# andimarafioti/faster-qwen3-tts

Hardware: AMD Instinct MI355X
Metric: real-time factor (audio s / wall s), Qwen3-TTS-12Hz-0.6B voice-clone streaming chunk_size=8; p50 TTFA in ttfa_ms_p50 (higher is better)
Workload: dtype bf16

## Files before the change

### faster-qwen3-tts_amd/csrc/decode_kernels.cuh

```cuda
#pragma once
#include "fq3_common.cuh"

namespace fq3 {

enum { PRO_PLAIN = 0, PRO_NORM = 1, PRO_COMBINE = 2 };
enum { EPI_STORE = 0, EPI_RESIDUAL = 1, EPI_SWIGLU = 2 };

constexpr int kHeadDim = 128;
constexpr int kKeysPerTile = 64;
constexpr int kMaxWorkers = 8;
constexpr int kPartStride = kHeadDim + 4;


struct GemvArgs {
    const void* W; int N; int K;
    const void* x;
    const void* norm_w; float eps;
    const void* bias;
    void* y;
    const void* res;
    void* xn_out;
    int up_off;
    const float* part; int n_part; int rep;
    const void* x2; void* y2; const void* res2; size_t part_stride2;
// ... 352 lines not shown
        l[h] = xrow_sum(l[h] * w);
#pragma unroll
        for (int i = 0; i < 8; ++i) o[h][i] = xrow_sum(o[h][i] * w);
        m[h] = M;
    }
    if (sub == 0) {
#pragma unroll
        for (int h = 0; h < REP; ++h) {
#pragma unroll
            for (int i = 0; i < 8; ++i) wo[wave][h][c * 8 + i] = o[h][i];
            if (c == 0) { wm[wave][h] = m[h]; wl[wave][h] = l[h]; }
        }
    }
    __syncthreads();
    for (int e = tid; e < REP * HD; e += 256) {
        const int h = e / HD, d = e - h * HD;
        float M = fmaxf(fmaxf(wm[0][h], wm[1][h]), fmaxf(wm[2][h], wm[3][h]));
        float num = 0.f, den = 0.f;
#pragma unroll
        for (int w = 0; w < 4; ++w) {
            const float ww = __expf(wm[w][h] - M);
            num = fmaf(ww, wo[w][h][d], num);
            den = fmaf(ww, wl[w][h], den);
        }
        float* p = a.part + (((size_t)g * kMaxWorkers + s) * REP + h) * kPartStride;
        p[d] = num;
        if (d == 0) { p[HD] = M; p[HD + 1] = den; }
    }
}

template <typename T, int REP, bool PAGED>
__global__ __launch_bounds__(256) void attn_decode_kernel(AttnArgs a) { attn_decode_body<T, REP, PAGED>(a); }

template <typename T>
__device__ __forceinline__ void attn_pred_body(const AttnArgs& a, int head) {
    constexpr int HD = kHeadDim;
    const int g = head / a.rep, hh = head - g * a.rep;
    const int lane = threadIdx.x & 63, sub = lane >> 4, c = lane & 15;
    const int pos = a.pos_imm;
    const T* qkv = reinterpret_cast<const T*>(a.qkv);
    const int q_dim = a.n_kv * a.rep * HD, kv_dim = a.n_kv * HD;
    T* kc = reinterpret_cast<T*>(a.kcache) + (size_t)g * a.max_seq * HD;
    T* vc = reinterpret_cast<T*>(a.vcache) + (size_t)g * a.max_seq * HD;
    Raw8<T> qraw, knraw, vnraw, qwraw, kwraw, kr[4], vr[4];
    ldraw<false>(qraw, qkv + (size_t)head * HD + c * 8);
    ldraw<false>(knraw, qkv + q_dim + (size_t)g * HD + c * 8);
    ldraw<false>(vnraw, qkv + q_dim + kv_dim + (size_t)g * HD + c * 8);
    ldraw<false>(qwraw, reinterpret_cast<const T*>(a.q_norm_w) + c * 8);
    ldraw<false>(kwraw, reinterpret_cast<const T*>(a.k_norm_w) + c * 8);
    const f32x4 cs0 = *reinterpret_cast<const f32x4*>(a.cos_row + ((c * 8) & 63)), cs1 = *reinterpret_cast<const f32x4*>(a.cos_row + ((c * 8 + 4) & 63));
    const f32x4 sn0 = *reinterpret_cast<const f32x4*>(a.sin_row + ((c * 8) & 63)), sn1 = *reinterpret_cast<const f32x4*>(a.sin_row + ((c * 8 + 4) & 63));
#pragma unroll
    for (int i = 0; i < 4; ++i) {
        int key = i * 4 + sub;
        key = key < a.max_seq ? key : a.max_seq - 1;
        ldraw<false>(kr[i], kc + (size_t)key * HD + c * 8);
        ldraw<false>(vr[i], vc + (size_t)key * HD + c * 8);
    }
    __builtin_amdgcn_sched_barrier(0);
    const float sgn = c < 8 ? -1.f : 1.f;
    const float cs[8] = {cs0.x, cs0.y, cs0.z, cs0.w, cs1.x, cs1.y, cs1.z, cs1.w};
    const float sn[8] = {sgn * sn0.x, sgn * sn0.y, sgn * sn0.z, sgn * sn0.w, sgn * sn1.x, sgn * sn1.y, sgn * sn1.z, sgn * sn1.w};
    auto norm_rope = [&](const Raw8<T>& raw, const Raw8<T>& wraw, float (&out)[8]) {
        float x[8], w[8];
        unpack(raw, x); unpack(wraw, w);
        float ss = 0.f;
#pragma unroll
        for (int i = 0; i < 8; ++i) ss = fmaf(x[i], x[i], ss);
        ss = row16_sum(ss);
        const float rs = 1.0f / sqrtf(ss / (float)HD + a.eps);
#pragma unroll
        for (int i = 0; i < 8; i += 2) {
            float u = x[i] * rs, v = x[i + 1] * rs;
            DT<T>::rnd2(u, v);
            u *= w[i]; v *= w[i + 1];
            DT<T>::rnd2(u, v);
            x[i] = u; x[i + 1] = v;
        }
#pragma unroll
        for (int i = 0; i < 8; i += 2) {
            float a0 = x[i] * cs[i], a1 = x[i + 1] * cs[i + 1];
            float b0 = row16_xor8(x[i]) * sn[i], b1 = row16_xor8(x[i + 1]) * sn[i + 1];
            DT<T>::rnd2(a0, a1); DT<T>::rnd2(b0, b1);
            float r0 = a0 + b0, r1 = a1 + b1;
            DT<T>::rnd2(r0, r1);
            out[i] = r0; out[i + 1] = r1;
        }
    };
    float qr[8], knew[8], vnew[8];
    norm_rope(qraw, qwraw, qr);
    norm_rope(knraw, kwraw, knew);
    unpack(vnraw, vnew);
    if (hh == 0 && sub == 0) {
        DT<T>::st8(kc + (size_t)pos * HD + c * 8, knew);
        DT<T>::st8(vc + (size_t)pos * HD + c * 8, vnew);
    }
    float sc[5];
#pragma unroll
    for (int i = 0; i < 4; ++i) {
        float kf[8], s = 0.f;
        unpack(kr[i], kf);
#pragma unroll
        for (int d = 0; d < 8; ++d) s = fmaf(qr[d], kf[d], s);
        s = row16_sum(s);
        sc[i] = (i * 4 + sub < pos) ? s * a.scale : -INFINITY;
    }
    {
        float s = 0.f;
#pragma unroll
        for (int d = 0; d < 8; ++d) s = fmaf(qr[d], knew[d], s);
        s = row16_sum(s);
        sc[4] = sub == 0 ? s * a.scale : -INFINITY;
    }
    const float mx = wave_max(fmaxf(fmaxf(fmaxf(sc[0], sc[1]), fmaxf(sc[2], sc[3])), sc[4]));
    float p[5], lsum = 0.f, o[8];
#pragma unroll
    for (int i = 0; i < 5; ++i) { p[i] = __expf(sc[i] - mx); lsum += p[i]; }
    lsum = wave_sum(lsum) * (1.0f / 16.0f);
#pragma unroll
    for (int d = 0; d < 8; ++d) o[d] = p[4] * vnew[d];
#pragma unroll
    for (int i = 0; i < 4; ++i) {
        float vf[8];
        if (!(i * 4 + sub < pos)) zero(vr[i]);
        unpack(vr[i], vf);
#pragma unroll
        for (int d = 0; d < 8; ++d) o[d] = fmaf(p[i], vf[d], o[d]);
    }
    const float inv = 1.0f / lsum;
#pragma unroll
    for (int d = 0; d < 8; ++d) o[d] = xrow_sum(o[d]) * inv;
    if (sub == 0) DT<T>::st8(reinterpret_cast<T*>(a.out) + (size_t)head * HD + c * 8, o);
}

// ... 79 lines not shown
            float s = 0.f;
#pragma unroll
            for (int d = 0; d < 8; ++d) s = fmaf(qr[d], kf[i][d], s);
            s = row16_sum(s);
            sc[i] = (i * 4 + sub < pos) ? s * a.scale : -INFINITY;
        }
        {
            float s = 0.f;
#pragma unroll
            for (int d = 0; d < 8; ++d) s = fmaf(qr[d], knew[d], s);
            s = row16_sum(s);
            sc[4] = sub == 0 ? s * a.scale : -INFINITY;
        }
        const float mx = wave_max(fmaxf(fmaxf(fmaxf(sc[0], sc[1]), fmaxf(sc[2], sc[3])), sc[4]));
        float p[5], lsum = 0.f, o[8];
#pragma unroll
        for (int i = 0; i < 5; ++i) { p[i] = __expf(sc[i] - mx); lsum += p[i]; }
        lsum = wave_sum(lsum) * (1.0f / 16.0f);
#pragma unroll
        for (int d = 0; d < 8; ++d) o[d] = p[4] * vnew[d];
#pragma unroll
        for (int i = 0; i < 4; ++i)
#pragma unroll
            for (int d = 0; d < 8; ++d) o[d] = fmaf(p[i], vf[i][d], o[d]);
        const float inv = 1.0f / lsum;
#pragma unroll
        for (int d = 0; d < 8; ++d) o[d] = xrow_sum(o[d]) * inv;
        if (sub == 0) DT<T>::st8(reinterpret_cast<T*>(a.out) + (size_t)(g * REP + h) * HD + c * 8, o);
    }
}

template <typename T>
__global__ __launch_bounds__(64) void attn_pred_kernel(AttnArgs a) { attn_pred_body<T>(a); }

template <typename T>
__global__ __launch_bounds__(256) void rmsnorm_kernel(const T* x, const T* w, T* y, int K, float eps) {
    __shared__ float red[8];
    float ss = 0.f;
    for (int e = threadIdx.x; e < K; e += 256) { const float v = DT<T>::ld(x + e); ss = fmaf(v, v, ss); }
    ss = block_sum<4>(ss, red);
    const float rs = 1.0f / sqrtf(ss / (float)K + eps);
    for (int e = threadIdx.x; e < K; e += 256)
        DT<T>::st(y + e, DT<T>::ld(w + e) * DT<T>::rnd(DT<T>::ld(x + e) * rs));
}

template <typename T>
__global__ void copy_kernel(T* dst, const T* src, int n) {
    const int i = blockIdx.x * blockDim.x + threadIdx.x;
    if (i < n) dst[i] = src[i];
}

struct DecodeState {
    int token, frame, pos, gen_step, done;
    int min_new, max_new, trailing_len, noise_frames, eos_id, max_seq, sup_lo, sup_hi;
    float t_temperature; int t_top_k; float t_top_p; int t_do_sample; float t_rep_penalty;
    float p_temperature; int p_top_k; float p_top_p; int p_do_sample;
    const void* trailing_text; const void* tts_pad; const void* talker_noise; const void* pred_noise;
    const void* past_hidden_init;
    int n_pad, rope_delta;
};

struct TeacherForcing { const int* forced; int* decisions; };

__device__ __forceinline__ int forced_or(const TeacherForcing* tf, int slot, int tok) {
    if (!tf) return tok;
    const int* forced = gptr(tf->forced); int* dec = gptr(tf->decisions);
    if (dec && threadIdx.x == 0) dec[slot] = tok;
    return forced ? forced[slot] : tok;
}

template <typename T>
__device__ __forceinline__ void frame_begin_body(DecodeState* st, const T* codec_emb, const T* past_hidden,
                                                 T* pred_in, int* codes, unsigned char* seen, int H, int G) {
    if (st->done) return;
    const int tok = st->token;
    if (tok == st->eos_id || st->frame >= st->max_new) {
        __syncthreads();
        if (threadIdx.x == 0) st->done = 1;
        return;
    }
    if (threadIdx.x == 0) { codes[(size_t)st->frame * G] = tok; seen[tok] = 1; }
    for (int e = threadIdx.x; e < H; e += 256) {
        pred_in[e] = past_hidden[e];
        pred_in[H + e] = codec_emb[(size_t)tok * H + e];
    }
}
template <typename T>
__global__ __launch_bounds__(256) void frame_begin_kernel(DecodeState* st, const T* codec_emb, const T* past_hidden,
                                                          T* pred_in, int* codes, unsigned char* seen, int H, int G) {
    frame_begin_body<T>(st, codec_emb, past_hidden, pred_in, codes, seen, H, G);
}

struct EmbTables { const void* t[32]; };

template <typename T, int G>
__device__ __forceinline__ void embed_sum_body(DecodeState* st, const EmbTables& tabs, const int* codes, T* x, int H,
                                               const float* cos_tab, const float* sin_tab, int rope_len,
                                               int rope_delta, float* rope_now) {
    const int done = st->done, frame = st->frame, pos = st->pos, gen_step = st->gen_step;
    const int trailing_len = st->trailing_len, max_seq = st->max_seq;
    const T* trailing = gptr(reinterpret_cast<const T*>(st->trailing_text));
    const T* pad = gptr(reinterpret_cast<const T*>(st->tts_pad));
    if (done) return;
    if (pos >= max_seq - 1) {
        __syncthreads();
        if (threadIdx.x == 0) { st->frame = frame + 1; st->done = 1; }
        return;
    }
    int ids[G];
#pragma unroll
    for (int gI = 0; gI < G; ++gI) ids[gI] = codes[(size_t)frame * G + gI];
    if (threadIdx.x < kHeadDim) {
        int rp = pos + rope_delta;
        rp = rp < 0 ? 0 : (rp >= rope_len ? rope_len - 1 : rp);
        const int i = threadIdx.x & 63;
        rope_now[threadIdx.x] = threadIdx.x < 64 ? cos_tab[(size_t)rp * 64 + i] : sin_tab[(size_t)rp * 64 + i];
    }
    const T* text = gen_step < trailing_len ? trailing + (size_t)gen_step * H : pad;
    for (int e0 = threadIdx.x * 8; e0 < H; e0 += 256 * 8) {
        Raw8<T> r[G], tr;
#pragma unroll
        for (int gI = 0; gI < G; ++gI) ldraw<false>(r[gI], reinterpret_cast<const T*>(tabs.t[gI]) + (size_t)ids[gI] * H + e0);
        ldraw<false>(tr, text + e0);
        float sum[8], f[8];
        unpack(r[0], sum);
#pragma unroll
        for (int gI = 1; gI < G; ++gI) {
            unpack(r[gI], f);
#pragma unroll
            for (int i = 0; i < 8; ++i) sum[i] += f[i];
        }
        unpack(tr, f);
#pragma unroll
        for (int i = 0; i < 8; ++i) DT<T>::st(x + e0 + i, DT<T>::rnd(sum[i]) + f[i]);
    }
}
template <typename T, int G>
__global__ __launch_bounds__(256) void embed_sum_kernel(DecodeState* st, EmbTables tabs, const int* codes, T* x, int H,
                                                        const float* cos_tab, const float* sin_tab, int rope_len,
                                                        int rope_delta, float* rope_now) {
    embed_sum_body<T, G>(st, tabs, codes, x, H, cos_tab, sin_tab, rope_len, rope_delta, rope_now);
}

}
// ... 1 lines not shown
```

### faster-qwen3-tts_amd/csrc/fq3_api.hip

```cpp
#define FQ3_SKINNY_EXTERN
#include "fq3_ctx.h"
#include "sampler.cuh"
#include "sampler_wave.cuh"
#include "skinny_gemm.cuh"

#include <cstdio>
#include <cstdlib>
#include <cstring>
#include <map>
#include <string>
#include <type_traits>
#include <vector>

using namespace fq3;

static thread_local std::string g_err;
static int fail(int code, const std::string& m) { g_err = m; return code; }
int fq3_fail_(int code, const std::string& m) { return fail(code, m); }
#define HIPCHK(x) do { hipError_t e_ = (x); if (e_ != hipSuccess) return fail(FQ3_EHIP, std::string(#x) + ": " + hipGetErrorString(e_)); } while (0)

extern "C" const char* fq3_last_error(void) { return g_err.c_str(); }
extern "C" void fq3_set_error_(const char* msg) { g_err = msg ? msg : ""; }
extern "C" int fq3_abi_version(void) { return FQ3_ABI_VERSION; }

// ... 193 lines not shown
    if ((r = dmalloc(c, &c->act2, (size_t)Im * c->esz))) return r;
    if ((r = dmalloc(c, &c->pred_x2, (size_t)p.hidden * c->esz))) return r;
    if ((r = dmalloc(c, &c->xin, (size_t)Hm * c->esz))) return r;
    if ((r = dmalloc(c, &c->tmp_hidden, (size_t)Hm * c->esz))) return r;
    if ((r = dmalloc(c, &c->qkv, (size_t)qkvm * c->esz))) return r;
    if ((r = dmalloc(c, &c->act, (size_t)Im * c->esz))) return r;
    if ((r = dmalloc(c, &c->logits, (size_t)Vm * c->esz))) return r;
    if ((r = dmalloc(c, &c->past_hidden, (size_t)t.hidden * c->esz))) return r;
    if ((r = dmalloc(c, &c->pred_in, (size_t)2 * t.hidden * c->esz))) return r;
    if ((r = dmalloc(c, &c->pred_next, (size_t)t.hidden * c->esz))) return r;
    if ((r = dmalloc(c, &c->pred_x, (size_t)p.hidden * c->esz))) return r;
    if ((r = dmalloc(c, &c->plogits, (size_t)(G - 1) * p.vocab * c->esz))) return r;
    const int maxkv = std::max(t.n_kv_heads, p.n_kv_heads);
    c->part_stride = (size_t)maxkv * kMaxWorkers * 4 * kPartStride;
    if ((r = dmalloc(c, (void**)&c->part, 2 * c->part_stride * sizeof(float)))) return r;
    if ((r = dmalloc(c, (void**)&c->rope_now, 2 * 64 * sizeof(float)))) return r;
    if ((r = dmalloc(c, (void**)&c->seen_api, kMaxVocab))) return r;
    if ((r = dmalloc(c, (void**)&c->st, sizeof(DecodeState)))) return r;
    if ((r = dmalloc(c, (void**)&c->seen, kMaxVocab))) return r;
    if ((r = dmalloc(c, (void**)&c->codes, (size_t)(frames + 1) * G * sizeof(int)))) return r;
    if ((r = dmalloc(c, (void**)&c->ids64, (size_t)64 * sizeof(int64_t)))) return r;
    if ((r = dmalloc(c, (void**)&c->d_pemb, (size_t)64 * sizeof(void*)))) return r;
    HIPCHK(hipStreamCreateWithFlags(&c->cap_stream, hipStreamNonBlocking));
    return FQ3_OK;
}

extern "C" int fq3_set_option(fq3_ctx* c, const char* key, int value) {
    if (!c || !key) return fail(FQ3_EINVAL, "null argument");
    const std::string k(key);
    if (k == "weight_nt") c->opt_nt = value;
    else if (k == "pred_m2") c->opt_m2 = value;
    else if (k == "pred_attn") c->opt_pred_attn = value;
    else if (k == "rows_per_wave_max") c->opt_rmax = value;
    else if (k == "prefill_mode") c->prefill_mode = value;
    else if (k == "flash_prefill") c->opt_flash_prefill = value;
    else if (k == "flash_small") c->opt_flash_small = value;
    else if (k == "swiglu_tile") c->opt_swiglu_tile = value;
    else if (k == "packed_weights") c->opt_packed = value;
    else if (k == "skinny_gemm") c->opt_no_skinny = !value;
    else return fail(FQ3_EINVAL, "unknown option: " + k);
    fq3_graph_reset(c);
    return FQ3_OK;
}

extern "C" int fq3_graph_reset(fq3_ctx* c) {
    if (!c) return fail(FQ3_EINVAL, "null ctx");
    if (c->exec) { (void)hipGraphExecDestroy(c->exec); c->exec = nullptr; }
    if (c->graph) { (void)hipGraphDestroy(c->graph); c->graph = nullptr; }
    return FQ3_OK;
}

namespace {
struct PackedEntry { void* p; int refs; int N, K; };
std::mutex g_packed_mu;
std::map<std::pair<const void*, int>, PackedEntry> g_packed;
}
const void* fq3_packed_find_(const void* W, int kind) {
    std::lock_guard<std::mutex> lk(g_packed_mu);
    auto it = g_packed.find({W, kind});
    return it == g_packed.end() ? nullptr : it->second.p;
}
int fq3_packed_acquire_(const void* W, int N, int K, int kind) {
    if (!W || !skinny_pack_ok(N, K) || (kind == 1 && (N / 2) % 8) || (kind == 2 && N % 512)) return FQ3_EUNSUPPORTED;
    std::lock_guard<std::mutex> lk(g_packed_mu);
    auto it = g_packed.find({W, kind});
    if (it != g_packed.end()) {
// ... 199 lines not shown
            o.x = c->attn_out;
            if (int r = launch_gemv<PRO_PLAIN, EPI_RESIDUAL>(c, o, nt, s)) return r;
        } else {
            if (c->cfg.dtype == FQ3_BF16) launch_attn_t<bf16_t>(a, rep, kv.workers, s);
            else launch_attn_t<float>(a, rep, kv.workers, s);
            if (tail_skip) break;
            o.part = c->part; o.n_part = kv.workers;
            if (int r = launch_gemv<PRO_COMBINE, EPI_RESIDUAL>(c, o, nt, s)) return r;
        }
        GemvArgs m{};
        m.eps = d.rms_eps; m.W = w.gate_up; m.N = d.inter; m.K = d.hidden; m.x = c->h;
        m.norm_w = w.post_norm; m.y = c->act; m.up_off = d.inter;
        if (int r = launch_gemv<PRO_NORM, EPI_SWIGLU>(c, m, nt, s)) return r;
        GemvArgs dn{};
        dn.W = w.down; dn.N = d.hidden; dn.K = d.inter; dn.x = c->act; dn.y = c->h; dn.res = c->h;
        if (int r = launch_gemv<PRO_PLAIN, EPI_RESIDUAL>(c, dn, nt, s)) return r;
    }
    return 0;
}

static int run_predictor_pair(fq3_ctx* c, const void* x_a, const void* x_b, hipStream_t s) {
    const fq3_stack_dims& d = c->cfg.predictor;
    StackBufs& kv = c->pk;
    const int rep = d.n_heads / d.n_kv_heads;
    const int q_dim = d.n_heads * kHeadDim, kv_dim = d.n_kv_heads * kHeadDim;
    for (int i = 0; i < d.n_layers; ++i) {
        const fq3_layer_weights& w = c->pl[i];
        const void* xa = i == 0 ? x_a : c->h;
        const void* xb = i == 0 ? x_b : c->h2;
        GemvArgs g{};
        g.eps = d.rms_eps; g.W = w.qkv; g.N = q_dim + 2 * kv_dim; g.K = d.hidden; g.x = xa; g.x2 = xb;
        g.norm_w = w.input_norm; g.y = c->qkv; g.y2 = c->qkv2;
        if (int r = launch_gemv2<PRO_NORM, EPI_STORE>(c, g, s)) return r;
        for (int m = 0; m < 2; ++m) {
            AttnArgs a{};
            a.qkv = m == 0 ? c->qkv : c->qkv2; a.q_norm_w = w.q_norm; a.k_norm_w = w.k_norm; a.eps = d.rms_eps;
            a.cos_row = c->wt.pred_cos + (size_t)m * 64; a.sin_row = c->wt.pred_sin + (size_t)m * 64;
            a.kcache = kv.k[i]; a.vcache = kv.v[i]; a.max_seq = kv.max_seq;
            a.pos_ptr = nullptr; a.pos_imm = m; a.n_pad = 0; a.n_kv = d.n_kv_heads;
            a.part = c->part + (size_t)m * c->part_stride; a.scale = 1.0f / sqrtf((float)kHeadDim);
            a.rep = rep; a.out = m == 0 ? c->attn_out : c->attn_out2;
            if (c->opt_pred_attn) {
                if (c->cfg.dtype == FQ3_BF16) hipLaunchKernelGGL((attn_pred_kernel<bf16_t>), dim3(d.n_heads), dim3(64), 0, s, a);
                else hipLaunchKernelGGL((attn_pred_kernel<float>), dim3(d.n_heads), dim3(64), 0, s, a);
            } else if (c->cfg.dtype == FQ3_BF16) launch_attn_t<bf16_t>(a, rep, kv.workers, s);
            else launch_attn_t<float>(a, rep, kv.workers, s);
        }
        GemvArgs o{};
        o.W = w.o; o.N = d.hidden; o.K = q_dim; o.y = c->h; o.y2 = c->h2; o.res = xa; o.res2 = xb; o.rep = rep;
        if (c->opt_pred_attn) {
            o.x = c->attn_out; o.x2 = c->attn_out2;
            if (int r = launch_gemv2<PRO_PLAIN, EPI_RESIDUAL>(c, o, s)) return r;
        } else {
            o.part = c->part; o.part_stride2 = c->part_stride; o.n_part = kv.workers;
            if (int r = launch_gemv2<PRO_COMBINE, EPI_RESIDUAL>(c, o, s)) return r;
        }
        GemvArgs m{};
        m.eps = d.rms_eps; m.W = w.gate_up; m.N = d.inter; m.K = d.hidden; m.x = c->h; m.x2 = c->h2;
        m.norm_w = w.post_norm; m.y = c->act; m.y2 = c->act2; m.up_off = d.inter;
        if (int r = launch_gemv2<PRO_NORM, EPI_SWIGLU>(c, m, s)) return r;
        GemvArgs dn{};
        dn.W = w.down; dn.N = d.hidden; dn.K = d.inter; dn.x = c->act; dn.x2 = c->act2; dn.y = c->h; dn.y2 = c->h2;
        dn.res = c->h; dn.res2 = c->h2;
        if (int r = launch_gemv2<PRO_PLAIN, EPI_RESIDUAL>(c, dn, s)) return r;
    }
    return 0;
}

#define NEED_BOUND(c) do { if (!(c)) return fail(FQ3_EINVAL, "null ctx"); if (!(c)->bound) return fail(FQ3_ESTATE, "weights not bound"); } while (0)
#define LAUNCH_CHECK() HIPCHK(hipGetLastError())

extern "C" int fq3_set_generation_state(fq3_ctx* c, int n_pad, int rope_delta) {
    if (!c) return fail(FQ3_EINVAL, "null ctx");
    if (n_pad < 0 || n_pad >= c->cfg.max_seq_len) return fail(FQ3_EINVAL, "n_pad out of range");
    if (c->n_pad != n_pad || c->rope_delta != rope_delta) fq3_graph_reset(c);
// ... 303 lines not shown
    return FQ3_OK;
}

template <typename T>
__global__ __launch_bounds__(256) void rep_penalty_kernel(T* logits, int V, const unsigned char* seen, float penalty) {
    for (int i = threadIdx.x; i < V; i += 256) {
        if (!seen[i]) continue;
        const float v = DT<T>::ld(logits + i);
        DT<T>::st(logits + i, v > 0.f ? v / penalty : v * penalty);
    }
}
extern "C" int fq3_apply_repetition_penalty(fq3_ctx* c, void* logits, int V, const int64_t* history, int n_hist,
                                            float penalty, void* stream) {
    if (!c || !logits) return fail(FQ3_EINVAL, "null argument");
    if (V <= 0 || V > kMaxVocab) return fail(FQ3_EUNSUPPORTED, "vocab must be at most 4096");
    if (penalty == 1.0f || n_hist <= 0 || !history) return FQ3_OK;
    hipStream_t s = (hipStream_t)stream;
    hipLaunchKernelGGL(build_seen_kernel, dim3(1), dim3(256), 0, s, history, n_hist, c->seen_api, V);
    if (c->cfg.dtype == FQ3_BF16) hipLaunchKernelGGL((rep_penalty_kernel<bf16_t>), dim3(1), dim3(256), 0, s, (bf16_t*)logits, V, c->seen_api, penalty);
    else hipLaunchKernelGGL((rep_penalty_kernel<float>), dim3(1), dim3(256), 0, s, (float*)logits, V, c->seen_api, penalty);
    LAUNCH_CHECK();
    return FQ3_OK;
}

extern "C" int fq3_set_predictor_sampling(fq3_ctx* c, const fq3_sampling* s) {
    if (!c || !s) return fail(FQ3_EINVAL, "null argument");
    if (s->do_sample && !(s->temperature > 0.f)) return fail(FQ3_EINVAL, "temperature must be > 0");
    if ((s->top_p >= 1.0f) != (c->pred_sampling.top_p >= 1.0f)) fq3_graph_reset(c);
    c->pred_sampling = *s;
    return FQ3_OK;
}

template <typename T>
static int predictor_passes_t(fq3_ctx* c, const DecodeState* st_dev, const void* pred_input, const void* noise_imm,
                              int64_t* out64, void* out_logits, hipStream_t s) {
    const fq3_stack_dims &p = c->cfg.predictor, &t = c->cfg.talker;
    const int G = c->cfg.num_code_groups, Vp = p.vocab, Ht = t.hidden;
    SampleCfg scfg = to_cfg(c->pred_sampling);
    for (int pass = 0; pass < G; ++pass) {
        const void* hsrc = c->h;
        if (pass == 0 && c->opt_m2) {
            const T* xa = (const T*)pred_input;
            const T* xb = (const T*)pred_input + Ht;
            if (c->cfg.has_projection) {
                GemvArgs g{};
                g.W = c->wt.proj_w; g.bias = c->wt.proj_b; g.N = p.hidden; g.K = Ht; g.x = xa; g.x2 = xb; g.y = c->pred_x; g.y2 = c->pred_x2;
                if (int r = launch_gemv2<PRO_PLAIN, EPI_STORE>(c, g, s)) return r;
                xa = (const T*)c->pred_x; xb = (const T*)c->pred_x2;
            }
            if (int r = run_predictor_pair(c, xa, xb, s)) return r;
            pass = 1;
            hsrc = c->h2;
        } else {
        const T* x_talker = pass < 2 ? (const T*)pred_input + (size_t)pass * Ht : (const T*)c->pred_next;
        const void* x0 = x_talker;
        if (c->cfg.has_projection) {
            GemvArgs g{};
            g.W = c->wt.proj_w; g.bias = c->wt.proj_b; g.N = p.hidden; g.K = Ht; g.x = x_talker; g.y = c->pred_x;
            if (int r = launch_gemv<PRO_PLAIN, EPI_STORE>(c, g, false, s)) return r;
            x0 = c->pred_x;
        }
        StepSrc src{x0, nullptr, pass};
        src.kv_only_tail = pass == 0;
        if (int r = run_stack(c, false, src, s)) return r;
        }
        if (pass == 0) continue;
        const int cb = pass - 1;
        T* lg = out_logits ? (T*)out_logits + (size_t)cb * Vp : (T*)c->plogits + (size_t)cb * Vp;
        GemvArgs hgm{};
        hgm.eps = p.rms_eps; hgm.W = c->lmh[cb]; hgm.N = Vp; hgm.K = p.hidden; hgm.x = hsrc;
        hgm.norm_w = c->wt.predictor_final_norm; hgm.y = lg;
        if (int r = launch_gemv<PRO_NORM, EPI_STORE>(c, hgm, false, s)) return r;
        const T* nz = noise_imm ? (const T*)noise_imm + (size_t)cb * Vp : nullptr;
        const T* next_emb = cb + 1 < G - 1 ? (const T*)c->pemb[cb] : nullptr;
        launch_sample_pred<T>(st_dev, (const T*)lg, Vp, cb, scfg, nz, st_dev ? c->codes : nullptr, G, out64, next_emb,
                              (T*)c->pred_next, Ht, c->pred_sampling.top_p >= 1.0f, st_dev ? c->tf : nullptr, s);
    }
    return 0;
}

extern "C" int fq3_predictor_loop(fq3_ctx* c, const void* pred_input, const void* noise, int64_t* out_ids,
                                  void* out_logits, void* stream) {
    NEED_BOUND(c);
    if (!pred_input || !out_ids) return fail(FQ3_EINVAL, "null argument");
    if (c->pred_sampling.do_sample && !noise) return fail(FQ3_EINVAL, "predictor sampling enabled but no noise given");
    hipStream_t s = (hipStream_t)stream;
    int r = c->cfg.dtype == FQ3_BF16 ? predictor_passes_t<bf16_t>(c, nullptr, pred_input, noise, out_ids, out_logits, s)
                                     : predictor_passes_t<float>(c, nullptr, pred_input, noise, out_ids, out_logits, s);
    if (r) return r;
    LAUNCH_CHECK();
    return FQ3_OK;
}

__global__ __launch_bounds__(256) void decode_arm_kernel(DecodeState* st, DecodeState init, unsigned char* seen, int seen_bytes,
                                                         uint32_t* past_hidden, const uint32_t* ph_src, int ph_words) {
    for (int i = threadIdx.x; i < seen_bytes / 4; i += 256) reinterpret_cast<uint32_t*>(seen)[i] = 0u;
    for (int i = threadIdx.x; i < ph_words; i += 256) past_hidden[i] = ph_src[i];
    if (threadIdx.x == 0) *st = init;
}
__global__ void decode_set_forced_kernel(TeacherForcing* tf, const int* forced, int* decisions) {
    tf->forced = forced; tf->decisions = decisions;
}

extern "C" int fq3_decode_begin(fq3_ctx* c, const fq3_decode_params* p, void* stream) {
    NEED_BOUND(c);
    if (!p || !p->past_hidden || !p->tts_pad_embed) return fail(FQ3_EINVAL, "null argument");
    if (p->trailing_len > 0 && !p->trailing_text) return fail(FQ3_EINVAL, "trailing_text");
// ... 23 lines not shown
    hipLaunchKernelGGL(decode_arm_kernel, dim3(1), dim3(256), 0, s, c->st, h, c->seen, (int)kMaxVocab,
                       (uint32_t*)c->past_hidden, (const uint32_t*)p->past_hidden, (int)((size_t)c->cfg.talker.hidden * c->esz / 4));
    LAUNCH_CHECK();
    return FQ3_OK;
}

__global__ void decode_cancel_kernel(DecodeState* st) { st->done = 1; }
extern "C" int fq3_decode_cancel(fq3_ctx* c, void* stream) {
    if (!c) return fail(FQ3_EINVAL, "null ctx");
    hipLaunchKernelGGL(decode_cancel_kernel, dim3(1), dim3(1), 0, (hipStream_t)stream, c->st);
    LAUNCH_CHECK();
    return FQ3_OK;
}

extern "C" int fq3_decode_set_forced(fq3_ctx* c, const int32_t* forced_codes, int32_t* decisions, void* stream) {
    NEED_BOUND(c);
    if (!c->tf) {
        if (!forced_codes && !decisions) return FQ3_OK;
        if (int r = dmalloc(c, (void**)&c->tf, sizeof(TeacherForcing))) return r;
        fq3_graph_reset(c);
    }
    hipLaunchKernelGGL(decode_set_forced_kernel, dim3(1), dim3(1), 0, (hipStream_t)stream, c->tf, forced_codes, decisions);
    LAUNCH_CHECK();
    return FQ3_OK;
}

template <typename T>
static int enqueue_frame_t(fq3_ctx* c, hipStream_t s) {
    const fq3_stack_dims& t = c->cfg.talker;
    const int G = c->cfg.num_code_groups, H = t.hidden;
    DecodeState* st = c->st;
    hipLaunchKernelGGL((frame_begin_kernel<T>), dim3(1), dim3(256), 0, s, st, (const T*)c->wt.codec_embedding,
                       (const T*)c->past_hidden, (T*)c->pred_in, c->codes, c->seen, H, G);
    if (int r = predictor_passes_t<T>(c, st, c->pred_in, nullptr, nullptr, nullptr, s)) return r;
    EmbTables tabs{};
    tabs.t[0] = c->wt.codec_embedding;
    for (int i = 1; i < G; ++i) tabs.t[i] = c->pemb[i - 1];
    if (G != 16) return fail(FQ3_EUNSUPPORTED, "the fused loop is built for 16 code groups");
    hipLaunchKernelGGL((embed_sum_kernel<T, 16>), dim3(1), dim3(256), 0, s, st, tabs, c->codes, (T*)c->xin, H,
                       c->wt.talker_cos, c->wt.talker_sin, c->wt.talker_rope_len, c->rope_delta, c->rope_now);
    StepSrc src{c->xin, &st->pos, 0};
    if (int r = run_stack(c, true, src, s)) return r;
    GemvArgs g{};
    g.eps = t.rms_eps; g.W = c->wt.codec_head; g.N = t.vocab; g.K = H; g.x = c->h;
    g.norm_w = c->wt.talker_final_norm; g.y = c->logits; g.xn_out = c->past_hidden;
    if (int r = launch_gemv<PRO_NORM, EPI_STORE>(c, g, true, s)) return r;
    launch_sample_talker<T>(st, (const T*)c->logits, t.vocab, c->seen, G, c->talker_wave, c->tf, s);
    return 0;
}
static int enqueue_frame(fq3_ctx* c, hipStream_t s) {
    return c->cfg.dtype == FQ3_BF16 ? enqueue_frame_t<bf16_t>(c, s) : enqueue_frame_t<float>(c, s);
}

extern "C" int fq3_graph_capture(fq3_ctx* c, void* stream) {
    NEED_BOUND(c);
    if (c->exec) return FQ3_OK;
    (void)stream;
    hipStream_t cs = c->cap_stream;
    HIPCHK(hipStreamBeginCapture(cs, hipStreamCaptureModeRelaxed));
    int r = enqueue_frame(c, cs);
    hipGraph_t g = nullptr;
    hipError_t e = hipStreamEndCapture(cs, &g);
    if (r) { if (g) (void)hipGraphDestroy(g); return r; }
    if (e != hipSuccess) return fail(FQ3_EHIP, std::string("hipStreamEndCapture: ") + hipGetErrorString(e));
    c->graph = g;
    HIPCHK(hipGraphInstantiate(&c->exec, c->graph, nullptr, nullptr, 0));
    return FQ3_OK;
}

extern "C" int fq3_decode_frames(fq3_ctx* c, int n_frames, void* stream) {
    NEED_BOUND(c);
    hipStream_t s = (hipStream_t)stream;
    for (int i = 0; i < n_frames; ++i) {
// ... 34 lines not shown
```

### faster-qwen3-tts_amd/csrc/fq3_ctx.h

```cpp
#pragma once
#include "../../include/fq3hip.h"
#include "decode_kernels.cuh"
#include <hip/hip_runtime.h>
#include <mutex>
#include <string>
#include <utility>
#include <vector>

struct fq3_kv_pool {
    int dtype = 0, esz = 2, n_layers = 0, n_kv = 0, n_blocks = 0;
    size_t blk_elems = 0;
    std::vector<void*> k, v;
    std::vector<int> free_list;
    std::mutex mu;
    int in_use_high = 0;
    int users = 0;
    bool is_private = false;
};

struct StackBufs {
    std::vector<void*> k, v;
    int max_seq = 0, workers = 1;
    fq3_kv_pool* pool = nullptr;
    int* d_table = nullptr;
    std::vector<int> blocks;
    int max_blocks = 0;
};

struct fq3_ctx {
    fq3_config cfg{};
    int esz = 2;
    std::vector<fq3_layer_weights> tl, pl;
    fq3_weight_table wt{};
    std::vector<const void*> pemb, lmh;
    const void** d_pemb = nullptr;
    bool bound = false;
    StackBufs tk, pk;
    void *h = nullptr, *xin = nullptr, *qkv = nullptr, *act = nullptr, *logits = nullptr, *past_hidden = nullptr;
    void *pred_in = nullptr, *pred_x = nullptr, *pred_next = nullptr, *plogits = nullptr, *tmp_hidden = nullptr;
    void *attn_out = nullptr, *attn_out2 = nullptr;
    void *h2 = nullptr, *qkv2 = nullptr, *act2 = nullptr, *pred_x2 = nullptr;
    size_t part_stride = 0;
    float* part = nullptr;
    float* rope_now = nullptr;
    unsigned char* seen_api = nullptr;
    fq3::DecodeState* st = nullptr;
    fq3::TeacherForcing* tf = nullptr;
    unsigned char* seen = nullptr;
    int* codes = nullptr;
    int64_t* ids64 = nullptr;
    int n_pad = 0, rope_delta = 0;
    int opt_nt = 1;
    int opt_m2 = 1;
    int opt_pred_attn = 1;
    int opt_rmax = 2;
    int opt_flash_prefill = 1;
    int opt_flash_small = 1;
    int opt_swiglu_tile = 1;
    int opt_packed = 1;
    std::vector<std::pair<const void*, int>> packed_refs;
    int opt_no_skinny = 0;
    int prefill_mode = 0;
    bool talker_wave = true;
    fq3_sampling pred_sampling{0.9f, 50, 1.0f, 1, 1.0f};
    hipGraph_t graph = nullptr;
    hipGraphExec_t exec = nullptr;
    hipStream_t cap_stream = nullptr;
    std::vector<void*> allocs;
    fq3_prompt_weights pw{};
    bool pw_bound = false;
    void *pw_x = nullptr, *pw_h = nullptr;
    int pw_cap = 0;
    void *pf_x = nullptr, *pf_xn = nullptr, *pf_qkv = nullptr, *pf_att = nullptr, *pf_gu = nullptr, *pf_act = nullptr, *pf_ws = nullptr;
};


const void* fq3_packed_find_(const void* W, int kind);
int fq3_packed_acquire_(const void* W, int N, int K, int kind);
void fq3_packed_release_(const void* W, int kind);

int fq3_fail_(int code, const std::string& m);
int fq3_kv_ensure_(fq3_ctx* c, int n_pos, hipStream_t s);
int fq3_prefill_reserve_(fq3_ctx* c);
int fq3_prefill_mfma_(fq3_ctx* c, const void* embeds, int L, int n_pad, void* out_logits, void* out_hidden, hipStream_t s);
int fq3_prefill_batch_mfma_(fq3_ctx* const* cs, int n, const void* const* embeds, const int* L, const int* n_pad, void* const* out_logits,
                            void* const* out_hidden, hipStream_t s);
int fq3_codec_head_launch_(fq3_ctx* c, const void* hidden, void* out_logits, hipStream_t s);
int fq3_dmalloc_(fq3_ctx* c, void** p, size_t bytes);
// ... 1 lines not shown
```

### faster-qwen3-tts_amd/csrc/sampler_wave.cuh

```cuda
#pragma once
#include "sampler.cuh"

namespace fq3 {

__device__ __forceinline__ ArgMax wave_argmax(ArgMax a) {
    ArgMax r;
    r.v = wave_max(a.v);
    r.i = wave_min_i32(a.v == r.v ? a.i : 0x7fffffff);
    return r;
}

struct BlkSmem { int cnt[2][4]; float f[4]; float av[4]; int ai[4]; };

__device__ __forceinline__ float blk_max4(float v, BlkSmem& sm) {
    v = wave_max(v);
    __syncthreads();
    if ((threadIdx.x & 63) == 0) sm.f[threadIdx.x >> 6] = v;
    __syncthreads();
    return fmaxf(fmaxf(sm.f[0], sm.f[1]), fmaxf(sm.f[2], sm.f[3]));
}
__device__ __forceinline__ float blk_sum4(float v, BlkSmem& sm) {
    v = wave_sum(v);
    __syncthreads();
    if ((threadIdx.x & 63) == 0) sm.f[threadIdx.x >> 6] = v;
// ... 119 lines not shown
    }
}

template <typename T, int NC>
__global__ __launch_bounds__(256) void sample_api_wave_kernel(const T* logits, int V, SampleCfg c, const unsigned char* seen,
                                                             const T* noise, int64_t* out) {
    __shared__ BlkSmem sm;
    Raw8<T> xraw[NC];
    issue_logits<T, NC>(xraw, logits, V);
    const int tok = sample_wave_core<T, NC>(xraw, V, c, seen, noise, sm);
    if (threadIdx.x == 0) out[0] = tok;
}

template <typename T, int NC>
__device__ __forceinline__ int sample_nucleus_from_regs(Raw8<T> (&xraw)[NC], int V, const SampleCfg& c, const unsigned char* seen,
                                                        const T* noise, SampleSmem& big) {
#pragma unroll
    for (int j = 0; j < NC; ++j) {
        float f[8];
        unpack(xraw[j], f);
#pragma unroll
        for (int i = 0; i < 8; ++i) {
            const int id = j * 2048 + threadIdx.x * 8 + i;
            if (id < V) big.vals[id] = f[i];
        }
    }
    __syncthreads();
    const int tok = sample_core<T>(big, V, c, seen, noise);
    __syncthreads();
    return tok;
}

template <typename T, int NC, bool NUCLEUS = false>
__device__ __forceinline__ void sample_pred_wave_body(const DecodeState* st, const T* logits, int V, int cb,
                                                      const SampleCfg& c_imm, const T* noise_imm, int* codes, int G,
                                                      int64_t* out64, const T* next_emb, T* next_in, int H, const TeacherForcing* tf = nullptr) {
    __shared__ BlkSmem sm;
    Raw8<T> xraw[NC];
    issue_logits<T, NC>(xraw, logits, V);
    SampleCfg c = c_imm;
    const T* noise = noise_imm;
    int frame = 0;
    if (st) {
        if (st->done) return;
        c.temperature = st->p_temperature; c.top_k = st->p_top_k; c.top_p = st->p_top_p; c.do_sample = st->p_do_sample;
        frame = st->frame;
        if (st->pred_noise)
            noise = gptr(reinterpret_cast<const T*>(st->pred_noise)) + ((size_t)(frame % st->noise_frames) * (G - 1) + cb) * V;
    }
    int tok;
    if constexpr (NUCLEUS) {
        __shared__ SampleSmem big;
        if (c.do_sample && c.top_p < 1.0f) tok = sample_nucleus_from_regs<T, NC>(xraw, V, c, nullptr, noise, big);
        else tok = sample_wave_core<T, NC>(xraw, V, c, nullptr, noise, sm);
    } else {
        tok = sample_wave_core<T, NC>(xraw, V, c, nullptr, noise, sm);
    }
    if (st) tok = forced_or(tf, frame * G + 1 + cb, tok);
    if (threadIdx.x == 0) {
        if (codes) codes[(size_t)frame * G + 1 + cb] = tok;
        if (out64) out64[cb] = tok;
    }
    if (next_emb) {
        const T* src = next_emb + (size_t)tok * H;
        for (int e = threadIdx.x * 8; e < H; e += 256 * 8) {
            Raw8<T> r; ldraw<false>(r, src + e);
            if (sizeof(T) == 2) *reinterpret_cast<u32x4*>(reinterpret_cast<char*>(next_in) + (size_t)e * 2) = *reinterpret_cast<u32x4*>(&r);
            else { float f[8]; unpack(r, f);
#pragma unroll
                   for (int i = 0; i < 8; ++i) DT<T>::st(next_in + e + i, f[i]); }
        }
    }
}

template <typename T, int NC>
__global__ __launch_bounds__(256) void sample_pred_wave_kernel(const DecodeState* st, const T* logits, int V, int cb,
                                                              SampleCfg c_imm, const T* noise_imm, int* codes, int G,
                                                              int64_t* out64, const T* next_emb, T* next_in, int H, const TeacherForcing* tf) {
    sample_pred_wave_body<T, NC>(st, logits, V, cb, c_imm, noise_imm, codes, G, out64, next_emb, next_in, H, tf);
}

template <typename T, int NC, bool NUCLEUS = false>
__device__ __forceinline__ void sample_talker_wave_body(DecodeState* st, const T* logits, int V, const unsigned char* seen, int G,
                                                        const TeacherForcing* tf = nullptr) {
    __shared__ BlkSmem sm;
    Raw8<T> xraw[NC];
    issue_logits<T, NC>(xraw, logits, V);
    if (st->done) return;
    SampleCfg c;
    c.temperature = st->t_temperature; c.top_k = st->t_top_k; c.top_p = st->t_top_p; c.do_sample = st->t_do_sample;
    c.rep_penalty = st->t_rep_penalty;
    c.sup_lo = st->sup_lo; c.sup_hi = st->sup_hi; c.keep_id = st->eos_id;
    const int frame = st->frame;
    c.sup_extra = (frame + 1 < st->min_new) ? st->eos_id : -1;
    const T* noise = st->talker_noise
        ? gptr(reinterpret_cast<const T*>(st->talker_noise)) + (size_t)(frame % st->noise_frames) * V : nullptr;
    int tok;
    if constexpr (NUCLEUS) {
        __shared__ SampleSmem big;
        if (c.do_sample && c.top_p < 1.0f) tok = sample_nucleus_from_regs<T, NC>(xraw, V, c, seen, noise, big);
        else tok = sample_wave_core<T, NC>(xraw, V, c, seen, noise, sm);
    } else {
        tok = sample_wave_core<T, NC>(xraw, V, c, seen, noise, sm);
    }
    tok = forced_or(tf, (frame + 1) * G, tok);
    if (threadIdx.x == 0) { st->token = tok; st->frame = frame + 1; st->pos += 1; st->gen_step += 1; }
}
template <typename T, int NC>
__global__ __launch_bounds__(256) void sample_talker_wave_kernel(DecodeState* st, const T* logits, int V,
                                                                const unsigned char* seen, int G, const TeacherForcing* tf) {
    sample_talker_wave_body<T, NC>(st, logits, V, seen, G, tf);
}
// ... 3 lines not shown
```

Before: 36.68.

## Fuse predictor two-step attention into one launch and merge last sample with embed sum

In the predictor's two-token prefill, the two attention launches are merged into one pair kernel. Its second grid row reads the first token's K/V straight from the first qkv buffer and recomputes their norm and RoPE, instead of waiting for the cache write. Separately, the final codebook sampling kernel now also performs the talker embedding sum, passing the sampled token in directly, which removes one kernel launch per frame. The trade-off is extra recomputation of the first token's K norm/RoPE and more complex kernels, plus a dependence on top_p>=1 for the merge path.

Result: no change. 36.71 (median of 5 runs) (+0.1%).

```diff
diff --git a/faster-qwen3-tts_amd/csrc/decode_kernels.cuh b/faster-qwen3-tts_amd/csrc/decode_kernels.cuh
--- a/faster-qwen3-tts_amd/csrc/decode_kernels.cuh
+++ b/faster-qwen3-tts_amd/csrc/decode_kernels.cuh
@@ -408,8 +408,8 @@
 template <typename T, int REP, bool PAGED>
 __global__ __launch_bounds__(256) void attn_decode_kernel(AttnArgs a) { attn_decode_body<T, REP, PAGED>(a); }
 
-template <typename T>
-__device__ __forceinline__ void attn_pred_body(const AttnArgs& a, int head) {
+template <typename T, bool SECOND = false>
+__device__ __forceinline__ void attn_pred_body(const AttnArgs& a, int head, const AttnArgs* first = nullptr) {
     constexpr int HD = kHeadDim;
     const int g = head / a.rep, hh = head - g * a.rep;
     const int lane = threadIdx.x & 63, sub = lane >> 4, c = lane & 15;
@@ -426,18 +426,31 @@
     ldraw<false>(kwraw, reinterpret_cast<const T*>(a.k_norm_w) + c * 8);
     const f32x4 cs0 = *reinterpret_cast<const f32x4*>(a.cos_row + ((c * 8) & 63)), cs1 = *reinterpret_cast<const f32x4*>(a.cos_row + ((c * 8 + 4) & 63));
     const f32x4 sn0 = *reinterpret_cast<const f32x4*>(a.sin_row + ((c * 8) & 63)), sn1 = *reinterpret_cast<const f32x4*>(a.sin_row + ((c * 8 + 4) & 63));
-#pragma unroll
-    for (int i = 0; i < 4; ++i) {
-        int key = i * 4 + sub;
-        key = key < a.max_seq ? key : a.max_seq - 1;
-        ldraw<false>(kr[i], kc + (size_t)key * HD + c * 8);
-        ldraw<false>(vr[i], vc + (size_t)key * HD + c * 8);
+    f32x4 fc0 = cs0, fc1 = cs1, fs0 = sn0, fs1 = sn1;
+    if constexpr (SECOND) {
+        const T* qkv0 = reinterpret_cast<const T*>(first->qkv);
+        ldraw<false>(kr[0], qkv0 + q_dim + (size_t)g * HD + c * 8);
+        ldraw<false>(vr[0], qkv0 + q_dim + kv_dim + (size_t)g * HD + c * 8);
+        fc0 = *reinterpret_cast<const f32x4*>(first->cos_row + ((c * 8) & 63)); fc1 = *reinterpret_cast<const f32x4*>(first->cos_row + ((c * 8 + 4) & 63));
+        fs0 = *reinterpret_cast<const f32x4*>(first->sin_row + ((c * 8) & 63)); fs1 = *reinterpret_cast<const f32x4*>(first->sin_row + ((c * 8 + 4) & 63));
+#pragma unroll
+        for (int i = 1; i < 4; ++i) { zero(kr[i]); zero(vr[i]); }
+    } else {
+#pragma unroll
+        for (int i = 0; i < 4; ++i) {
+            int key = i * 4 + sub;
+            key = key < a.max_seq ? key : a.max_seq - 1;
+            ldraw<false>(kr[i], kc + (size_t)key * HD + c * 8);
+            ldraw<false>(vr[i], vc + (size_t)key * HD + c * 8);
+        }
     }
     __builtin_amdgcn_sched_barrier(0);
     const float sgn = c < 8 ? -1.f : 1.f;
-    const float cs[8] = {cs0.x, cs0.y, cs0.z, cs0.w, cs1.x, cs1.y, cs1.z, cs1.w};
-    const float sn[8] = {sgn * sn0.x, sgn * sn0.y, sgn * sn0.z, sgn * sn0.w, sgn * sn1.x, sgn * sn1.y, sgn * sn1.z, sgn * sn1.w};
-    auto norm_rope = [&](const Raw8<T>& raw, const Raw8<T>& wraw, float (&out)[8]) {
+    const float cs_now[8] = {cs0.x, cs0.y, cs0.z, cs0.w, cs1.x, cs1.y, cs1.z, cs1.w};
+    const float sn_now[8] = {sgn * sn0.x, sgn * sn0.y, sgn * sn0.z, sgn * sn0.w, sgn * sn1.x, sgn * sn1.y, sgn * sn1.z, sgn * sn1.w};
+    const float cs_first[8] = {fc0.x, fc0.y, fc0.z, fc0.w, fc1.x, fc1.y, fc1.z, fc1.w};
+    const float sn_first[8] = {sgn * fs0.x, sgn * fs0.y, sgn * fs0.z, sgn * fs0.w, sgn * fs1.x, sgn * fs1.y, sgn * fs1.z, sgn * fs1.w};
+    auto norm_rope_at = [&](const Raw8<T>& raw, const Raw8<T>& wraw, const float (&cs)[8], const float (&sn)[8], float (&out)[8]) {
         float x[8], w[8];
         unpack(raw, x); unpack(wraw, w);
         float ss = 0.f;
@@ -463,9 +476,11 @@
             out[i] = r0; out[i + 1] = r1;
         }
     };
-    float qr[8], knew[8], vnew[8];
+    auto norm_rope = [&](const Raw8<T>& raw, const Raw8<T>& wraw, float (&out)[8]) { norm_rope_at(raw, wraw, cs_now, sn_now, out); };
+    float qr[8], knew[8], vnew[8], kfirst[8];
     norm_rope(qraw, qwraw, qr);
     norm_rope(knraw, kwraw, knew);
+    if constexpr (SECOND) norm_rope_at(kr[0], kwraw, cs_first, sn_first, kfirst);
     unpack(vnraw, vnew);
     if (hh == 0 && sub == 0) {
         DT<T>::st8(kc + (size_t)pos * HD + c * 8, knew);
@@ -476,6 +491,10 @@
     for (int i = 0; i < 4; ++i) {
         float kf[8], s = 0.f;
         unpack(kr[i], kf);
+        if constexpr (SECOND) if (i == 0) {
+#pragma unroll
+            for (int d = 0; d < 8; ++d) kf[d] = kfirst[d];
+        }
 #pragma unroll
         for (int d = 0; d < 8; ++d) s = fmaf(qr[d], kf[d], s);
         s = row16_sum(s);
@@ -621,6 +640,11 @@
 
 template <typename T>
 __global__ __launch_bounds__(64) void attn_pred_kernel(AttnArgs a) { attn_pred_body<T>(a); }
+template <typename T>
+__global__ __launch_bounds__(64) void attn_pred_pair_kernel(AttnArgs a0, AttnArgs a1) {
+    if (blockIdx.y == 0) attn_pred_body<T>(a0, (int)blockIdx.x);
+    else attn_pred_body<T, true>(a1, (int)blockIdx.x, &a0);
+}
 
 template <typename T>
 __global__ __launch_bounds__(256) void rmsnorm_kernel(const T* x, const T* w, T* y, int K, float eps) {
@@ -685,7 +709,7 @@
 template <typename T, int G>
 __device__ __forceinline__ void embed_sum_body(DecodeState* st, const EmbTables& tabs, const int* codes, T* x, int H,
                                                const float* cos_tab, const float* sin_tab, int rope_len,
-                                               int rope_delta, float* rope_now) {
+                                               int rope_delta, float* rope_now, int last_tok = -1) {
     const int done = st->done, frame = st->frame, pos = st->pos, gen_step = st->gen_step;
     const int trailing_len = st->trailing_len, max_seq = st->max_seq;
     const T* trailing = gptr(reinterpret_cast<const T*>(st->trailing_text));
@@ -699,6 +723,7 @@
     int ids[G];
 #pragma unroll
     for (int gI = 0; gI < G; ++gI) ids[gI] = codes[(size_t)frame * G + gI];
+    if (last_tok >= 0) ids[G - 1] = last_tok;
     if (threadIdx.x < kHeadDim) {
         int rp = pos + rope_delta;
         rp = rp < 0 ? 0 : (rp >= rope_len ? rope_len - 1 : rp);
diff --git a/faster-qwen3-tts_amd/csrc/fq3_api.hip b/faster-qwen3-tts_amd/csrc/fq3_api.hip
--- a/faster-qwen3-tts_amd/csrc/fq3_api.hip
+++ b/faster-qwen3-tts_amd/csrc/fq3_api.hip
@@ -249,6 +249,8 @@
     else if (k == "pred_m2") c->opt_m2 = value;
     else if (k == "pred_attn") c->opt_pred_attn = value;
     else if (k == "rows_per_wave_max") c->opt_rmax = value;
+    else if (k == "pred_attn_pair") c->opt_pred_attn_pair = value;
+    else if (k == "embed_merge") c->opt_embed_merge = value;
     else if (k == "prefill_mode") c->prefill_mode = value;
     else if (k == "flash_prefill") c->opt_flash_prefill = value;
     else if (k == "flash_small") c->opt_flash_small = value;
@@ -514,6 +516,7 @@
         g.eps = d.rms_eps; g.W = w.qkv; g.N = q_dim + 2 * kv_dim; g.K = d.hidden; g.x = xa; g.x2 = xb;
         g.norm_w = w.input_norm; g.y = c->qkv; g.y2 = c->qkv2;
         if (int r = launch_gemv2<PRO_NORM, EPI_STORE>(c, g, s)) return r;
+        AttnArgs pair[2];
         for (int m = 0; m < 2; ++m) {
             AttnArgs a{};
             a.qkv = m == 0 ? c->qkv : c->qkv2; a.q_norm_w = w.q_norm; a.k_norm_w = w.k_norm; a.eps = d.rms_eps;
@@ -522,7 +525,12 @@
             a.pos_ptr = nullptr; a.pos_imm = m; a.n_pad = 0; a.n_kv = d.n_kv_heads;
             a.part = c->part + (size_t)m * c->part_stride; a.scale = 1.0f / sqrtf((float)kHeadDim);
             a.rep = rep; a.out = m == 0 ? c->attn_out : c->attn_out2;
-            if (c->opt_pred_attn) {
+            pair[m] = a;
+            if (c->opt_pred_attn && c->opt_pred_attn_pair) {
+                if (m == 0) continue;
+                if (c->cfg.dtype == FQ3_BF16) hipLaunchKernelGGL((attn_pred_pair_kernel<bf16_t>), dim3(d.n_heads, 2), dim3(64), 0, s, pair[0], pair[1]);
+                else hipLaunchKernelGGL((attn_pred_pair_kernel<float>), dim3(d.n_heads, 2), dim3(64), 0, s, pair[0], pair[1]);
+            } else if (c->opt_pred_attn) {
                 if (c->cfg.dtype == FQ3_BF16) hipLaunchKernelGGL((attn_pred_kernel<bf16_t>), dim3(d.n_heads), dim3(64), 0, s, a);
                 else hipLaunchKernelGGL((attn_pred_kernel<float>), dim3(d.n_heads), dim3(64), 0, s, a);
             } else if (c->cfg.dtype == FQ3_BF16) launch_attn_t<bf16_t>(a, rep, kv.workers, s);
@@ -892,8 +900,8 @@
 }
 
 template <typename T>
-static int predictor_passes_t(fq3_ctx* c, const DecodeState* st_dev, const void* pred_input, const void* noise_imm,
-                              int64_t* out64, void* out_logits, hipStream_t s) {
+static int predictor_passes_t(fq3_ctx* c, DecodeState* st_dev, const void* pred_input, const void* noise_imm,
+                              int64_t* out64, void* out_logits, hipStream_t s, const EmbedSumArgs* embed = nullptr) {
     const fq3_stack_dims &p = c->cfg.predictor, &t = c->cfg.talker;
     const int G = c->cfg.num_code_groups, Vp = p.vocab, Ht = t.hidden;
     SampleCfg scfg = to_cfg(c->pred_sampling);
@@ -933,6 +941,14 @@
         if (int r = launch_gemv<PRO_NORM, EPI_STORE>(c, hgm, false, s)) return r;
         const T* nz = noise_imm ? (const T*)noise_imm + (size_t)cb * Vp : nullptr;
         const T* next_emb = cb + 1 < G - 1 ? (const T*)c->pemb[cb] : nullptr;
+        if (embed && cb == G - 2) {
+            dispatch_nc(Vp, [&](auto nc) {
+                constexpr int NC = decltype(nc)::value;
+                hipLaunchKernelGGL((sample_pred_embed_kernel<T, NC>), dim3(1), dim3(256), 0, s, st_dev, (const T*)lg, Vp, cb, scfg,
+                                   c->codes, Ht, c->tf, *embed);
+            });
+            continue;
+        }
         launch_sample_pred<T>(st_dev, (const T*)lg, Vp, cb, scfg, nz, st_dev ? c->codes : nullptr, G, out64, next_emb,
                               (T*)c->pred_next, Ht, c->pred_sampling.top_p >= 1.0f, st_dev ? c->tf : nullptr, s);
     }
@@ -1022,13 +1038,17 @@
     DecodeState* st = c->st;
     hipLaunchKernelGGL((frame_begin_kernel<T>), dim3(1), dim3(256), 0, s, st, (const T*)c->wt.codec_embedding,
                        (const T*)c->past_hidden, (T*)c->pred_in, c->codes, c->seen, H, G);
-    if (int r = predictor_passes_t<T>(c, st, c->pred_in, nullptr, nullptr, nullptr, s)) return r;
-    EmbTables tabs{};
-    tabs.t[0] = c->wt.codec_embedding;
-    for (int i = 1; i < G; ++i) tabs.t[i] = c->pemb[i - 1];
     if (G != 16) return fail(FQ3_EUNSUPPORTED, "the fused loop is built for 16 code groups");
-    hipLaunchKernelGGL((embed_sum_kernel<T, 16>), dim3(1), dim3(256), 0, s, st, tabs, c->codes, (T*)c->xin, H,
-                       c->wt.talker_cos, c->wt.talker_sin, c->wt.talker_rope_len, c->rope_delta, c->rope_now);
+    EmbedSumArgs es{};
+    es.tabs.t[0] = c->wt.codec_embedding;
+    for (int i = 1; i < G; ++i) es.tabs.t[i] = c->pemb[i - 1];
+    es.x = c->xin; es.cos_tab = c->wt.talker_cos; es.sin_tab = c->wt.talker_sin; es.rope_len = c->wt.talker_rope_len;
+    es.rope_delta = c->rope_delta; es.rope_now = c->rope_now;
+    const bool merged = c->opt_embed_merge && c->pred_sampling.top_p >= 1.0f;
+    if (int r = predictor_passes_t<T>(c, st, c->pred_in, nullptr, nullptr, nullptr, s, merged ? &es : nullptr)) return r;
+    if (!merged)
+        hipLaunchKernelGGL((embed_sum_kernel<T, 16>), dim3(1), dim3(256), 0, s, st, es.tabs, c->codes, (T*)c->xin, H,
+                           es.cos_tab, es.sin_tab, es.rope_len, es.rope_delta, es.rope_now);
     StepSrc src{c->xin, &st->pos, 0};
     if (int r = run_stack(c, true, src, s)) return r;
     GemvArgs g{};
diff --git a/faster-qwen3-tts_amd/csrc/fq3_ctx.h b/faster-qwen3-tts_amd/csrc/fq3_ctx.h
--- a/faster-qwen3-tts_amd/csrc/fq3_ctx.h
+++ b/faster-qwen3-tts_amd/csrc/fq3_ctx.h
@@ -54,6 +54,8 @@
     int opt_m2 = 1;
     int opt_pred_attn = 1;
     int opt_rmax = 2;
+    int opt_pred_attn_pair = 1;
+    int opt_embed_merge = 1;
     int opt_flash_prefill = 1;
     int opt_flash_small = 1;
     int opt_swiglu_tile = 1;
diff --git a/faster-qwen3-tts_amd/csrc/sampler_wave.cuh b/faster-qwen3-tts_amd/csrc/sampler_wave.cuh
--- a/faster-qwen3-tts_amd/csrc/sampler_wave.cuh
+++ b/faster-qwen3-tts_amd/csrc/sampler_wave.cuh
@@ -175,9 +175,9 @@
 }
 
 template <typename T, int NC, bool NUCLEUS = false>
-__device__ __forceinline__ void sample_pred_wave_body(const DecodeState* st, const T* logits, int V, int cb,
-                                                      const SampleCfg& c_imm, const T* noise_imm, int* codes, int G,
-                                                      int64_t* out64, const T* next_emb, T* next_in, int H, const TeacherForcing* tf = nullptr) {
+__device__ __forceinline__ int sample_pred_wave_body(const DecodeState* st, const T* logits, int V, int cb,
+                                                     const SampleCfg& c_imm, const T* noise_imm, int* codes, int G,
+                                                     int64_t* out64, const T* next_emb, T* next_in, int H, const TeacherForcing* tf = nullptr) {
     __shared__ BlkSmem sm;
     Raw8<T> xraw[NC];
     issue_logits<T, NC>(xraw, logits, V);
@@ -185,7 +185,7 @@
     const T* noise = noise_imm;
     int frame = 0;
     if (st) {
-        if (st->done) return;
+        if (st->done) return -1;
         c.temperature = st->p_temperature; c.top_k = st->p_top_k; c.top_p = st->p_top_p; c.do_sample = st->p_do_sample;
         frame = st->frame;
         if (st->pred_noise)
@@ -214,6 +214,7 @@
                    for (int i = 0; i < 8; ++i) DT<T>::st(next_in + e + i, f[i]); }
         }
     }
+    return tok;
 }
 
 template <typename T, int NC>
@@ -221,6 +222,17 @@
                                                               SampleCfg c_imm, const T* noise_imm, int* codes, int G,
                                                               int64_t* out64, const T* next_emb, T* next_in, int H, const TeacherForcing* tf) {
     sample_pred_wave_body<T, NC>(st, logits, V, cb, c_imm, noise_imm, codes, G, out64, next_emb, next_in, H, tf);
+}
+
+struct EmbedSumArgs {
+    EmbTables tabs; void* x; const float* cos_tab; const float* sin_tab; int rope_len, rope_delta; float* rope_now;
+};
+template <typename T, int NC>
+__global__ __launch_bounds__(256) void sample_pred_embed_kernel(DecodeState* st, const T* logits, int V, int cb, SampleCfg c_imm,
+                                                               int* codes, int H, const TeacherForcing* tf, EmbedSumArgs es) {
+    const int tok = sample_pred_wave_body<T, NC>(st, logits, V, cb, c_imm, (const T*)nullptr, codes, 16, (int64_t*)nullptr,
+                                                 (const T*)nullptr, (T*)nullptr, H, tf);
+    embed_sum_body<T, 16>(st, es.tabs, codes, (T*)es.x, H, es.cos_tab, es.sin_tab, es.rope_len, es.rope_delta, es.rope_now, tok);
 }
 
 template <typename T, int NC, bool NUCLEUS = false>
```
